# f-dangel/vivit

Measured on AMD Instinct MI355X. Metric: GGN eigenpairs/sec (Gram build + symeig), MLP 784-512-10, batch=4096, higher is better.
Workload: dtype f32

## Files before the change

### vivit_amd/csrc/sy2sb.hip

```cpp
#include <cstdlib>

#include "common.h"
#include "device_utils.h"
#include "eig_internal.h"

namespace vivit {

constexpr int SNB = 64;
constexpr int QT = 128;
constexpr int SGRP = 8;

__global__ __launch_bounds__(256) void sb_panel_load_kernel(const float *__restrict__ A, int64_t lda, int64_t j0, int64_t mp,
                                                            float *__restrict__ pan) {
  const int64_t idx = (int64_t)blockIdx.x * 256 + threadIdx.x;
  if (idx >= mp * SNB) return;
  const int64_t r = idx / SNB, c = idx - r * SNB;
  pan[idx] = A[(j0 + SNB + r) * lda + j0 + c];
}

__global__ __launch_bounds__(256) void sb_panel_load_row_kernel(const float *__restrict__ A, int64_t lda, int64_t j0, int64_t mp,
                                                                float *__restrict__ pan) {
  __shared__ float t[SNB][SNB + 1];
  const int64_t r0 = (int64_t)blockIdx.x * SNB;
  const int tid = threadIdx.x;
  for (int idx = tid; idx < SNB * SNB; idx += 256) {
    const int c = idx / SNB, rr = idx % SNB;
    t[c][rr] = r0 + rr < mp ? A[(j0 + c) * lda + j0 + SNB + r0 + rr] : 0.f;
  }
  __syncthreads();
  for (int idx = tid; idx < SNB * SNB; idx += 256) {
    const int rr = idx / SNB, c = idx % SNB;
    if (r0 + rr < mp) pan[(r0 + rr) * SNB + c] = t[c][rr];
  }
}

__global__ __launch_bounds__(256) void coef_gather_kernel(const float *__restrict__ S, int64_t lds_, int64_t g, int kp,
                                                          float *__restrict__ Coef) {
  const int idx = blockIdx.x * 256 + threadIdx.x;
  if (idx >= SNB * kp) return;
  const int k = idx / SNB, m = idx % SNB;
  Coef[(int64_t)m * kp + k] = S[(int64_t)k * lds_ + g + m];
}


__global__ __launch_bounds__(256) void qr_step_kernel(float *__restrict__ pan, int64_t mp, int c, int ncol, int nwg, QrPart pt,
                                                      float *__restrict__ vdst1, float *__restrict__ vdst2, int64_t lds_, int64_t gi0,
                                                      float *__restrict__ A, int64_t lda, int64_t j0,
                                                      float *__restrict__ tau1, float *__restrict__ betas) {
  __shared__ float tile[QT][SNB + 1];
  __shared__ float vs[QT], xs2[QT];
  __shared__ float zs[SNB];
  __shared__ float zq[4][SNB];
  __shared__ __attribute__((aligned(16))) float zq16[16][SNB];
  const int tid = threadIdx.x;
  const int64_t r0 = (int64_t)blockIdx.x * QT;
  constexpr int NTL = QT * (SNB / 4) / 256;
  float4 tl[NTL];
#pragma unroll
  for (int i = 0; i < NTL; ++i) {
    const int idx = tid + 256 * i;
    const int rl = idx / (SNB / 4), c4 = (idx - rl * (SNB / 4)) * 4;
    const int64_t r = r0 + rl;
    tl[i] = *reinterpret_cast<const float4 *>(pan + (r < mp ? r : 0) * SNB + c4);
  }
  const int par = c & 1;
  const float *uin = pt.u + (int64_t)par * nwg * SNB;
  const float *din = pt.diag + par * SNB;
  const int cq4 = tid & 15, q16 = tid >> 4;
  float4 pv[20];
#pragma unroll
  for (int i = 0; i < 20; ++i) {
    const int w = q16 + 16 * i;
    pv[i] = *reinterpret_cast<const float4 *>(uin + (int64_t)(w < nwg ? w : 0) * SNB + 4 * cq4);
  }
  const float din_c = din[c >= 0 ? c : 0], din_t = din[tid & (SNB - 1)];
  __builtin_amdgcn_sched_barrier(0);
#pragma unroll
  for (int i = 0; i < NTL; ++i) {
    const int idx = tid + 256 * i;
    const int rl = idx / (SNB / 4), c4 = (idx - rl * (SNB / 4)) * 4;
    const bool ok = r0 + rl < mp;
    tile[rl][c4 + 0] = ok ? tl[i].x : 0.f;
    tile[rl][c4 + 1] = ok ? tl[i].y : 0.f;
    tile[rl][c4 + 2] = ok ? tl[i].z : 0.f;
    tile[rl][c4 + 3] = ok ? tl[i].w : 0.f;
  }
  if (c >= 0) {
    {
      float4 acc = make_float4(0.f, 0.f, 0.f, 0.f);
#pragma unroll
      for (int i = 0; i < 20; ++i)
        if (q16 + 16 * i < nwg) { acc.x += pv[i].x; acc.y += pv[i].y; acc.z += pv[i].z; acc.w += pv[i].w; }
      for (int w0 = q16 + 16 * 20; w0 < nwg; w0 += 16 * 20) {
        float4 v[20];
#pragma unroll
        for (int i = 0; i < 20; ++i) {
          const int w = w0 + 16 * i;
          v[i] = *reinterpret_cast<const float4 *>(uin + (int64_t)(w < nwg ? w : 0) * SNB + 4 * cq4);
        }
#pragma unroll
        for (int i = 0; i < 20; ++i)
          if (w0 + 16 * i < nwg) { acc.x += v[i].x; acc.y += v[i].y; acc.z += v[i].z; acc.w += v[i].w; }
      }
      *reinterpret_cast<float4 *>(&zq16[q16][4 * cq4]) = acc;
    }
    __syncthreads();
    float ssq = 0.f;
#pragma unroll
    for (int g2 = 0; g2 < 16; ++g2) ssq += zq16[g2][c];
    const float alpha = din_c;
    float tau = 0.f, beta = alpha, scal = 0.f;
    if (ssq > 0.f) {
      beta = -copysignf(sqrt_nr(alpha * alpha + ssq), alpha);
      tau = (beta - alpha) * rcp_nr(beta);
      scal = rcp_nr(alpha - beta);
    }
    if (tid < SNB) {
      float u = 0.f;
#pragma unroll
      for (int g2 = 0; g2 < 16; ++g2) u += zq16[g2][tid];
      zs[tid] = tid > c ? tau * (din_t + scal * u) : 0.f;
    }
    if (tid < QT) {
      const int64_t r = r0 + tid;
      float v = 0.f;
      if (r < mp) {
        if (r == c) v = 1.f;
        else if (r > c) v = tile[tid][c] * scal;
        vdst1[(int64_t)c * lds_ + gi0 + r] = v;
        vdst2[(int64_t)c * lds_ + gi0 + r] = v;
        if (r >= c) A[(j0 + c) * lda + gi0 + r] = v;
      }
      vs[tid] = v;
    }
    if (blockIdx.x == 0 && tid == 0) { tau1[j0 + c] = tau; betas[c] = beta; }
  } else {
    if (tid < QT) vs[tid] = 0.f;
    if (tid < SNB) zs[tid] = 0.f;
  }
  __syncthreads();
  const int cn = c + 1;
  const bool has_next = cn < ncol;
  if (tid < QT) {
    const int64_t r = r0 + tid;
    xs2[tid] = (has_next && r > cn && r < mp) ? tile[tid][cn] - vs[tid] * zs[cn] : 0.f;
  }
  __syncthreads();
  {
    const int cc = tid & 63, q = tid >> 6;
    const float zc = zs[cc];
    float acc = 0.f;
#pragma unroll 8
    for (int i = 0; i < QT / 4; ++i) {
      const int rl = q + 4 * i;
      const float v = vs[rl];
      float x = tile[rl][cc];
      if (cc > c && v != 0.f) {
        x -= v * zc;
        tile[rl][cc] = x;
        if (r0 + rl < mp) pan[(r0 + rl) * SNB + cc] = x;
      }
      acc += xs2[rl] * x;
    }
    zq[q][cc] = acc;
  }
  if (!has_next) return;
  __syncthreads();
  {
    const int par = cn & 1;
    if (tid < SNB) pt.u[((int64_t)par * nwg + blockIdx.x) * SNB + tid] = (zq[0][tid] + zq[1][tid]) + (zq[2][tid] + zq[3][tid]);
    if (cn >= r0 && cn < r0 + QT && tid < SNB) pt.diag[par * SNB + tid] = tile[cn - r0][tid];
  }
}

constexpr int QP_WG = 32, QP_THREADS = 512;
struct QrPersistWs {
  float *ubuf;
  float *dbuf;
  int *counter;
  int *tmo;
  int attempt;
  int fault;
};

__device__ __forceinline__ float sel8(float a0, float a1, float a2, float a3, float a4, float a5, float a6, float a7, int j) {
  const float t0 = (j & 1) ? a1 : a0, t1 = (j & 1) ? a3 : a2, t2 = (j & 1) ? a5 : a4, t3 = (j & 1) ? a7 : a6;
  const float u0 = (j & 2) ? t1 : t0, u1 = (j & 2) ? t3 : t2;
  return (j & 4) ? u1 : u0;
}

template <int RI>
__global__ __launch_bounds__(QP_THREADS) void qr_persist_kernel(float *__restrict__ pan, int64_t mp, int ncol, QrPersistWs pw,
                                                                float *__restrict__ vdst1, float *__restrict__ vdst2, int64_t lds_,
                                                                int64_t gi0, float *__restrict__ A, int64_t lda, int64_t j0,
                                                                float *__restrict__ tau1, float *__restrict__ betas) {
  if ((blockIdx.x & 7) != 0) return;
  if (pw.attempt == 1 && __hip_atomic_load(pw.counter + 1, __ATOMIC_RELAXED, __HIP_MEMORY_SCOPE_AGENT) != PERSIST_ABORT) return;
  int *const cnt = pw.counter + 8 * pw.attempt;
  const int w = blockIdx.x >> 3;
  const int tid = threadIdx.x, lane = tid & 63, wave = tid >> 6;
  const int cg = tid & 7, rs = tid >> 3;
  constexpr int RW = 64 * RI;
  const int64_t rbase = (int64_t)w * RW;
  __shared__ float s_u[SNB], s_d[SNB], s_dn[SNB];
  __shared__ float s_red[QP_THREADS / 64][SNB];
  __shared__ float s_v[RW];
  __shared__ int s_flag[2];

  float x[RI][8];
#pragma unroll
  for (int i = 0; i < RI; ++i) {
    const int64_t r = rbase + rs + 64 * i;
    const float *src = pan + (r < mp ? r : 0) * SNB + 8 * cg;
    const float4 a = *reinterpret_cast<const float4 *>(src), b = *reinterpret_cast<const float4 *>(src + 4);
    const bool ok = r < mp;
    x[i][0] = ok ? a.x : 0.f; x[i][1] = ok ? a.y : 0.f; x[i][2] = ok ? a.z : 0.f; x[i][3] = ok ? a.w : 0.f;
    x[i][4] = ok ? b.x : 0.f; x[i][5] = ok ? b.y : 0.f; x[i][6] = ok ? b.z : 0.f; x[i][7] = ok ? b.w : 0.f;
  }
  if (tid == 0) {
    int xcc;
    __asm__ volatile("s_getreg_b32 %0, hwreg(HW_REG_XCC_ID)" : "=s"(xcc));
    __hip_atomic_store(pw.counter + 32 + w, xcc & 15, __ATOMIC_RELAXED, __HIP_MEMORY_SCOPE_AGENT);
    __asm__ volatile("s_waitcnt vmcnt(0)" ::: "memory");
    const bool go = persist_arrive(cnt, cnt + 1, QP_WG, ((pw.fault >> pw.attempt) & 1) ? 0ull : PERSIST_TIMEOUT_TICKS);
    const int dead = go ? 0 : 2;
    int slow = 0;
    const int x0 = __hip_atomic_load(pw.counter + 32, __ATOMIC_RELAXED, __HIP_MEMORY_SCOPE_AGENT);
    for (int i = 1; i < QP_WG; ++i) slow |= __hip_atomic_load(pw.counter + 32 + i, __ATOMIC_RELAXED, __HIP_MEMORY_SCOPE_AGENT) != x0;
    s_flag[0] = slow;
    s_flag[1] = dead;
  }
  __syncthreads();
  const bool slow = s_flag[0] != 0;
  if (s_flag[1] == 2) {
    if (tid == 0 && w == 0 && pw.attempt == 1) {
      __hip_atomic_fetch_or(pw.tmo, PERSIST_TMO_PANEL_QR, __ATOMIC_RELAXED, __HIP_MEMORY_SCOPE_AGENT);
      betas[0] = __builtin_nanf("");
    }
    return;
  }
  const int grp = lane & ~7;

  auto publish = [&](int cn) __attribute__((always_inline)) {
    float acc[8];
#pragma unroll
    for (int j = 0; j < 8; ++j) acc[j] = 0.f;
#pragma unroll
    for (int i = 0; i < RI; ++i) {
      const int64_t r = rbase + rs + 64 * i;
      float xn = __shfl(sel8(x[i][0], x[i][1], x[i][2], x[i][3], x[i][4], x[i][5], x[i][6], x[i][7], cn & 7), grp | (cn >> 3), 64);
      xn = (r > cn && r < mp) ? xn : 0.f;
#pragma unroll
      for (int j = 0; j < 8; ++j) acc[j] = fmaf(xn, x[i][j], acc[j]);
    }
#pragma unroll
    for (int j = 0; j < 8; ++j) {
      acc[j] += __shfl_xor(acc[j], 8, 64);
      acc[j] += __shfl_xor(acc[j], 16, 64);
      acc[j] += __shfl_xor(acc[j], 32, 64);
    }
    if (lane < 8) {
#pragma unroll
      for (int j = 0; j < 8; ++j) s_red[wave][8 * lane + j] = acc[j];
    }
    if (w == 0 && rs == cn) {
#pragma unroll
      for (int j = 0; j < 8; ++j) s_dn[8 * cg + j] = x[0][j];
    }
  };
  auto send = [&](int par) __attribute__((always_inline)) {
    if (wave == 0) {
      float u = 0.f;
#pragma unroll
      for (int q = 0; q < QP_THREADS / 64; ++q) u += s_red[q][lane];
      float *ub = pw.ubuf + ((size_t)par * QP_WG + w) * SNB + lane, *db = pw.dbuf + (size_t)par * SNB + lane;
      if (slow) {
        __hip_atomic_store(ub, u, __ATOMIC_RELAXED, __HIP_MEMORY_SCOPE_AGENT);
        if (w == 0) __hip_atomic_store(db, s_dn[lane], __ATOMIC_RELAXED, __HIP_MEMORY_SCOPE_AGENT);
      } else {
        *ub = u;
        if (w == 0) *db = s_dn[lane];
      }
      __asm__ volatile("s_waitcnt vmcnt(0)" ::: "memory");
      if (lane == 0) __hip_atomic_fetch_add(cnt, 1, __ATOMIC_RELAXED, __HIP_MEMORY_SCOPE_AGENT);
    }
  };

  publish(0);
  __syncthreads();
  send(0);
  for (int c = 0; c < ncol && !s_flag[1]; ++c) {
    const int par = c & 1;
    if (wave == 0) {
      const int target = (c + 2) * QP_WG;
      const unsigned long long t0 = __builtin_amdgcn_s_memrealtime();
      while (__hip_atomic_load(cnt, __ATOMIC_RELAXED, __HIP_MEMORY_SCOPE_AGENT) < target)
        if (__builtin_amdgcn_s_memrealtime() - t0 > PERSIST_TIMEOUT_TICKS) { s_flag[1] = 1; break; }
      const float *ub = pw.ubuf + (size_t)par * QP_WG * SNB + lane;
      float pv[QP_WG];
#pragma unroll
      for (int q = 0; q < QP_WG; ++q) pv[q] = __hip_atomic_load(ub + q * SNB, __ATOMIC_RELAXED, __HIP_MEMORY_SCOPE_AGENT);
      const float dn = __hip_atomic_load(pw.dbuf + (size_t)par * SNB + lane, __ATOMIC_RELAXED, __HIP_MEMORY_SCOPE_AGENT);
      float u = 0.f;
#pragma unroll
      for (int q = 0; q < QP_WG; ++q) u += pv[q];
      s_u[lane] = u;
      s_d[lane] = dn;
    }
    __syncthreads();
    if (s_flag[1]) break;
    const float ssq = s_u[c], alpha = s_d[c];
    float tau = 0.f, beta = alpha, scal = 0.f;
    if (ssq > 0.f) {
      beta = -copysignf(sqrt_nr(alpha * alpha + ssq), alpha);
      tau = (beta - alpha) * rcp_nr(beta);
      scal = rcp_nr(alpha - beta);
    }
    float z[8];
#pragma unroll
    for (int j = 0; j < 8; ++j) {
      const int cc = 8 * cg + j;
      z[j] = cc > c ? tau * (s_d[cc] + scal * s_u[cc]) : 0.f;
    }
#pragma unroll
    for (int i = 0; i < RI; ++i) {
      const int64_t r = rbase + rs + 64 * i;
      const float xc = __shfl(sel8(x[i][0], x[i][1], x[i][2], x[i][3], x[i][4], x[i][5], x[i][6], x[i][7], c & 7), grp | (c >> 3), 64);
      const float v = r == c ? 1.f : ((r > c && r < mp) ? xc * scal : 0.f);
      if (cg == 0) s_v[rs + 64 * i] = v;
#pragma unroll
      for (int j = 0; j < 8; ++j) x[i][j] = fmaf(-v, z[j], x[i][j]);
    }
    if (w == 0 && tid == 0) { tau1[j0 + c] = tau; betas[c] = beta; }
    const bool has_next = c + 1 < ncol;
    if (has_next) publish(c + 1);
    __syncthreads();
    if (has_next) send(par ^ 1);
    for (int idx = tid; idx < RW; idx += QP_THREADS) {
      const int64_t r = rbase + idx;
      if (r < mp) {
        const float v = s_v[idx];
        vdst1[(int64_t)c * lds_ + gi0 + r] = v;
        vdst2[(int64_t)c * lds_ + gi0 + r] = v;
        if (r >= c) A[(j0 + c) * lda + gi0 + r] = v;
      }
    }
  }
  if (w == 0) {
    const int64_t r = rs;
    if (r < mp) {
      float *dst = pan + r * SNB + 8 * cg;
      *reinterpret_cast<float4 *>(dst) = make_float4(x[0][0], x[0][1], x[0][2], x[0][3]);
      *reinterpret_cast<float4 *>(dst + 4) = make_float4(x[0][4], x[0][5], x[0][6], x[0][7]);
    }
    if (tid == 0 && s_flag[1]) {
      betas[0] = __builtin_nanf("");
      __hip_atomic_fetch_or(pw.tmo, PERSIST_TMO_PANEL_QR, __ATOMIC_RELAXED, __HIP_MEMORY_SCOPE_AGENT);
    }
  }
}

static bool qr_persist_enabled() {
  static int on = -1;
  if (on < 0) {
    const char *e = getenv("VIVIT_QR_PERSIST");
    on = e ? atoi(e) : 1;
  }
  return on != 0 && persist_override() != 0;
}
constexpr size_t QR_PERSIST_WS_BYTES = sizeof(float) * (2 * QP_WG * SNB + 2 * SNB) + 64 * sizeof(int) + 256;

static bool qr_persist_launch(float *pan, int64_t mp, int ncol, void *wsp, float *v1, float *v2, int64_t ldn, int64_t gi0, float *A,
                              int64_t lda, int64_t j0, float *tau1, float *betas, hipStream_t stream) {
  if (!qr_persist_enabled() || mp > (int64_t)QP_WG * 64 * 20 || device_cu_count() < 256) return false;
  QrPersistWs pw;
  pw.ubuf = reinterpret_cast<float *>(align_up(reinterpret_cast<uintptr_t>(wsp), 256));
  pw.dbuf = pw.ubuf + 2 * QP_WG * SNB;
  pw.counter = reinterpret_cast<int *>(pw.dbuf + 2 * SNB);
  pw.tmo = persist_timeout_word(stream);
  pw.fault = persist_fault();
  if (!pw.tmo) return false;
  if (hipMemsetAsync(pw.counter, 0, 64 * sizeof(int), stream) != hipSuccess) return false;
  const int64_t ri = cdiv(mp, (int64_t)QP_WG * 64);
  const dim3 grid(8 * QP_WG);
#define QP_LAUNCH(RI) qr_persist_kernel<RI><<<grid, QP_THREADS, 0, stream>>>(pan, mp, ncol, pw, v1, v2, ldn, gi0, A, lda, j0, tau1, betas)
  for (int attempt = 0; attempt < 2; ++attempt) {
    pw.attempt = attempt;
    if (ri <= 1) QP_LAUNCH(1);
    else if (ri <= 2) QP_LAUNCH(2);
    else if (ri <= 3) QP_LAUNCH(3);
    else if (ri <= 5) QP_LAUNCH(5);
    else if (ri <= 8) QP_LAUNCH(8);
    else if (ri <= 12) QP_LAUNCH(12);
    else if (ri <= 16) QP_LAUNCH(16);
    else QP_LAUNCH(20);
  }
#undef QP_LAUNCH
  return true;
}

struct Sk64Args {
  const float *Coef;
  const float *B;
  float *Out;
  int64_t ldcoef, ldb, ldo, N;
  int K;
  float alpha, beta;
};
constexpr int SK_LDC = 36, SK_COLS = 128, SK_LDB = SK_COLS + 4, SK_NT = SK_COLS / 64;

__global__ __launch_bounds__(256) void skinny64_kernel(Sk64Args p) {
  __shared__ __attribute__((aligned(16))) float sC[64 * SK_LDC];
  __shared__ __attribute__((aligned(16))) float sB[32 * SK_LDB];
  const int tid = threadIdx.x, lane = tid & 63, wave = tid >> 6;
  const int r = lane & 31, h = lane >> 5, wm = wave >> 1, wn = wave & 1;
  const int64_t c0 = (int64_t)blockIdx.x * SK_COLS;
  f32x16 acc[SK_NT];
#pragma unroll
  for (int t = 0; t < SK_NT; ++t)
#pragma unroll
    for (int e = 0; e < 16; ++e) acc[t][e] = 0.f;
  constexpr int NLB = 32 * SK_COLS / 4 / 256;
  float4 rc[2], rb[NLB];
  auto gload = [&](int k0) __attribute__((always_inline)) {
#pragma unroll
    for (int i = 0; i < 2; ++i) {
      const int idx = tid + 256 * i;
      const int m = idx >> 3, kq = (idx & 7) * 4;
      rc[i] = *reinterpret_cast<const float4 *>(p.Coef + (int64_t)m * p.ldcoef + k0 + kq);
    }
#pragma unroll
    for (int i = 0; i < NLB; ++i) {
      const int idx = tid + 256 * i;
      const int kr = idx / (SK_COLS / 4), cq = (idx % (SK_COLS / 4)) * 4;
      const int64_t c = c0 + cq;
      rb[i] = *reinterpret_cast<const float4 *>(p.B + (int64_t)(k0 + kr) * p.ldb + (c < p.N ? c : 0));
    }
    __builtin_amdgcn_sched_barrier(0);
  };
  gload(0);
  for (int k0 = 0; k0 < p.K; k0 += 32) {
    __syncthreads();
#pragma unroll
    for (int i = 0; i < 2; ++i) {
      const int idx = tid + 256 * i;
      *reinterpret_cast<float4 *>(sC + (idx >> 3) * SK_LDC + (idx & 7) * 4) = rc[i];
    }
#pragma unroll
    for (int i = 0; i < NLB; ++i) {
      const int idx = tid + 256 * i;
      const int kr = idx / (SK_COLS / 4), cq = (idx % (SK_COLS / 4)) * 4;
      *reinterpret_cast<float4 *>(sB + kr * SK_LDB + cq) = c0 + cq < p.N ? rb[i] : make_float4(0.f, 0.f, 0.f, 0.f);
    }
    __syncthreads();
    if (k0 + 32 < p.K) gload(k0 + 32);
    const float *pa = sC + (32 * wm + r) * SK_LDC + 4 * h;
#pragma unroll
    for (int j = 0; j < 4; ++j) {
      const float4 a4 = *reinterpret_cast<const float4 *>(pa + 8 * j);
      const float av[4] = {a4.x, a4.y, a4.z, a4.w};
      float bv[4][SK_NT];
#pragma unroll
      for (int i = 0; i < 4; ++i)
#pragma unroll
        for (int t = 0; t < SK_NT; ++t) bv[i][t] = sB[(8 * j + 4 * h + i) * SK_LDB + 64 * wn + 32 * t + r];
#pragma unroll
      for (int i = 0; i < 4; ++i)
#pragma unroll
        for (int t = 0; t < SK_NT; ++t) acc[t] = __builtin_amdgcn_mfma_f32_32x32x2f32(av[i], bv[i][t], acc[t], 0, 0, 0);
    }
  }
#pragma unroll
  for (int t = 0; t < SK_NT; ++t) {
    const int64_t c = c0 + 64 * wn + 32 * t + r;
    if (c < p.N) {
#pragma unroll
      for (int e = 0; e < 16; ++e) {
        const int m = 32 * wm + (e & 3) + 8 * (e >> 2) + 4 * h;
        float *o = p.Out + (int64_t)m * p.ldo + c;
        float v = p.alpha * acc[t][e];
        if (p.beta != 0.f) v += p.beta * *o;
        *o = v;
      }
    }
  }
}

static bool skinny64_launch(const float *Coef, int64_t ldcoef, const float *B, int64_t ldb, float *Out, int64_t ldo, int64_t N, int64_t K,
                            float alpha, float beta, hipStream_t stream) {
  if (K < 32 || K % 32 != 0 || K > 4096 || N % 4 != 0 || ldb % 4 != 0 || ldcoef % 4 != 0 ||
      (reinterpret_cast<uintptr_t>(Coef) & 15) || (reinterpret_cast<uintptr_t>(B) & 15))
    return false;
  Sk64Args a;
  a.Coef = Coef; a.B = B; a.Out = Out; a.ldcoef = ldcoef; a.ldb = ldb; a.ldo = ldo; a.N = N; a.K = (int)K; a.alpha = alpha; a.beta = beta;
  skinny64_kernel<<<(unsigned)cdiv(N, SK_COLS), 256, 0, stream>>>(a);
  return true;
}

__global__ __launch_bounds__(256) void w_coef_kernel(const float *__restrict__ T, const float *__restrict__ G, float *__restrict__ Coef) {
  __shared__ float sT[SNB][SNB + 1], sG[SNB][SNB + 1], sU[SNB][SNB + 1];
  const int tid = threadIdx.x, lane = tid & 63, wave = tid >> 6;
  const int r = lane & 31, h = lane >> 5, qi = (wave >> 1) * 32, qj = (wave & 1) * 32;
  for (int idx = tid; idx < SNB * SNB; idx += 256) {
    sT[idx / SNB][idx % SNB] = T[idx];
    sG[idx / SNB][idx % SNB] = G[idx];
  }
  __syncthreads();
  f32x16 acc;
#pragma unroll
  for (int e = 0; e < 16; ++e) acc[e] = 0.f;
#pragma unroll 8
  for (int s2 = 0; s2 < SNB / 2; ++s2) acc = __builtin_amdgcn_mfma_f32_32x32x2f32(sT[2 * s2 + h][qi + r], sG[2 * s2 + h][qj + r], acc, 0, 0, 0);
#pragma unroll
  for (int e = 0; e < 16; ++e) sU[qi + (e & 3) + 8 * (e >> 2) + 4 * h][qj + r] = acc[e];
  __syncthreads();
#pragma unroll
  for (int e = 0; e < 16; ++e) acc[e] = 0.f;
#pragma unroll 8
  for (int s2 = 0; s2 < SNB / 2; ++s2) acc = __builtin_amdgcn_mfma_f32_32x32x2f32(sU[qi + r][2 * s2 + h], sT[2 * s2 + h][qj + r], acc, 0, 0, 0);
#pragma unroll
  for (int e = 0; e < 16; ++e) {
    const int a_ = qi + (e & 3) + 8 * (e >> 2) + 4 * h, b_ = qj + r;
    Coef[a_ * 2 * SNB + b_] = -0.5f * acc[e];
    Coef[a_ * 2 * SNB + SNB + b_] = sT[b_][a_];
  }
}

__global__ __launch_bounds__(256) void sb_panel_store_kernel(float *__restrict__ A, int64_t lda, int64_t j0, int64_t mp,
                                                             const float *__restrict__ pan, const float *__restrict__ betas) {
  const int idx = blockIdx.x * 256 + threadIdx.x;
  if (idx >= SNB * SNB) return;
  const int r = idx / SNB, c = idx - r * SNB;
  if (r >= mp) return;
  A[(j0 + SNB + r) * lda + j0 + c] = (r < c) ? pan[(int64_t)r * SNB + c] : (r == c ? betas[c] : 0.f);
}

__global__ __launch_bounds__(256) void larft_kernel(const float *__restrict__ S, int64_t lds_, const float *__restrict__ tau, int nb,
                                                    int nvalid, float *__restrict__ T) {
  constexpr int H = SNB / 2, LD = SNB + 1;
  __shared__ float Ss[SNB * LD], Ts[SNB * LD], Xs[H * (H + 1)], taus[SNB];
  const int tid = threadIdx.x;
  for (int idx = tid; idx < SNB * SNB; idx += 256) {
    Ss[(idx / SNB) * LD + (idx % SNB)] = S[(int64_t)(idx / SNB) * lds_ + (idx % SNB)];
    Ts[(idx / SNB) * LD + (idx % SNB)] = 0.f;
  }
  if (tid < SNB) taus[tid] = (tid < nvalid && tid < nb) ? tau[tid] : 0.f;
  __syncthreads();
  if (tid < SNB) {
    const int half = tid / H, j = tid % H;
    const float *Sb = Ss + half * (H * LD + H), *tb = taus + half * H;
    float t[H];
#pragma unroll
    for (int c = 0; c < H; ++c) t[c] = 0.f;
#pragma unroll
    for (int i = H - 1; i >= 0; --i) {
      float acc = 0.f;
#pragma unroll
      for (int c = i + 1; c < H; ++c) acc += Sb[i * LD + c] * t[c];
      t[i] = i == j ? tb[j] : (i < j ? -tb[i] * acc : 0.f);
    }
    float *Tb = Ts + half * (H * LD + H);
#pragma unroll
    for (int i = 0; i < H; ++i) Tb[i * LD + j] = t[i];
  }
  __syncthreads();
  if (tid < 64) {
    const int r = tid & 31, h = tid >> 5;
    f32x16 acc;
#pragma unroll
    for (int e = 0; e < 16; ++e) acc[e] = 0.f;
#pragma unroll 8
    for (int s2 = 0; s2 < H / 2; ++s2)
      acc = __builtin_amdgcn_mfma_f32_32x32x2f32(Ss[r * LD + H + 2 * s2 + h], Ts[(H + 2 * s2 + h) * LD + H + r], acc, 0, 0, 0);
#pragma unroll
    for (int e = 0; e < 16; ++e) Xs[((e & 3) + 8 * (e >> 2) + 4 * h) * (H + 1) + r] = acc[e];
  }
  __syncthreads();
  if (tid < 64) {
    const int r = tid & 31, h = tid >> 5;
    f32x16 acc;
#pragma unroll
    for (int e = 0; e < 16; ++e) acc[e] = 0.f;
#pragma unroll 8
    for (int s2 = 0; s2 < H / 2; ++s2)
      acc = __builtin_amdgcn_mfma_f32_32x32x2f32(Ts[r * LD + 2 * s2 + h], Xs[(2 * s2 + h) * (H + 1) + r], acc, 0, 0, 0);
#pragma unroll
    for (int e = 0; e < 16; ++e) Ts[((e & 3) + 8 * (e >> 2) + 4 * h) * LD + H + r] = -acc[e];
  }
  __syncthreads();
  for (int idx = tid; idx < SNB * SNB; idx += 256) T[idx] = Ts[(idx / SNB) * LD + (idx % SNB)];
}

__global__ __launch_bounds__(256) void sb_extract_band_kernel(const float *__restrict__ A, int64_t lda, int64_t n,
                                                              float *__restrict__ AB, int64_t ldab) {
  const int64_t idx = (int64_t)blockIdx.x * 256 + threadIdx.x;
  if (idx >= n * ldab) return;
  const int64_t i = idx / ldab;
  const int d = (int)(idx - i * ldab);
  const int64_t j = i - 2 * SNB + d;
  AB[idx] = (d >= SNB && d <= 2 * SNB && j >= 0) ? A[i * lda + j] : 0.f;
}

static size_t sy2sb_gemm_ws_bytes(int64_t n) {
  size_t m = 0;
  for (int64_t mp = 1; mp <= n; mp = mp < 4096 ? mp * 2 : mp + 4096) {
    const int64_t q = mp < n ? mp : n;
    size_t a = gemm_workspace_bytes(SNB, SNB, q, false);
    size_t b = gemm_workspace_bytes(SNB, q, q, false);
    size_t c = gemm_workspace_bytes(SNB, q, SNB, false);
    size_t d = 0, e = 0, f = 0;
    for (int g = 1; g < SGRP; ++g) {
      const size_t d1 = gemm_workspace_bytes(SNB, 2 * SNB * g + SNB, q, false), e1 = gemm_workspace_bytes(SNB, q, 2 * SNB * g, false);
      const size_t f1 = gemm_workspace_bytes(q, SNB, 2 * SNB * g, false);
      d = d1 > d ? d1 : d; e = e1 > e ? e1 : e; f = f1 > f ? f1 : f;
    }
    m = a > m ? a : m; m = b > m ? b : m; m = c > m ? c : m;
    m = d > m ? d : m; m = e > m ? e : m; m = f > m ? f : m;
    const size_t u = gemm_workspace_bytes(q, q, (int64_t)2 * SNB * SGRP, true);
    m = u > m ? u : m;
  }
  size_t a = gemm_workspace_bytes(SNB, SNB, n, false), b = gemm_workspace_bytes(SNB, n, n, false);
  m = a > m ? a : m; m = b > m ? b : m;
  return m * 2;
}

Sy2sbWs sy2sb_layout(Arena &a, int64_t n) {
  const int64_t nwg = cdiv(n, QT) + 1;
  Sy2sbWs ws;
  ws.pan = a.take<float>(n * SNB);
  ws.stackA = a.take<float>(2 * SGRP * SNB * n);
  ws.stackB = a.take<float>(2 * SGRP * SNB * n);
  ws.xt = a.take<float>(SNB * n);
  ws.G12 = a.take<float>(SNB * 2 * SNB * SGRP);
  ws.qp.u = a.take<float>(2 * nwg * SNB);
  ws.qp.diag = a.take<float>(2 * SNB);
  ws.qpw = a.take<char>(QR_PERSIST_WS_BYTES);
  ws.S = a.take<float>(SNB * SNB);
  ws.T = a.take<float>(SNB * SNB);
  ws.Y3 = a.take<float>(SNB * SNB);
  ws.S2 = a.take<float>(SNB * SNB);
  ws.tau1 = a.take<float>(n);
  ws.betas = a.take<float>(SNB);
  ws.gws_bytes = sy2sb_gemm_ws_bytes(n);
  ws.gws = a.take<char>(ws.gws_bytes);
  return ws;
}

size_t sy2sb_workspace_bytes(int64_t n) {
  Arena m;
  sy2sb_layout(m, n);
  return m.used() + 1024;
}

int sy2sb_launch(float *A, int64_t n, int64_t lda, const Sy2sbWs &ws, hipStream_t stream) {
  if (hipMemsetAsync(ws.tau1, 0, sizeof(float) * n, stream) != hipSuccess) return VIVIT_E_LAUNCH;

  const int64_t ldn = n;
  const bool rowmode = (n % 4 == 0) && (lda % 4 == 0) && (reinterpret_cast<uintptr_t>(A) & 15) == 0;
  auto factor_panel = [&](int64_t j0, float *v1, float *v2) -> int {
    const int64_t mp = n - j0 - SNB, gi0 = j0 + SNB;
    const int ncol = (int)(mp < SNB ? mp : SNB);
    const int g = (int)cdiv(mp, QT);
    if (rowmode) sb_panel_load_row_kernel<<<(unsigned)cdiv(mp, SNB), 256, 0, stream>>>(A, lda, j0, mp, ws.pan);
    else sb_panel_load_kernel<<<(unsigned)cdiv(mp * SNB, 256), 256, 0, stream>>>(A, lda, j0, mp, ws.pan);
    if (!qr_persist_launch(ws.pan, mp, ncol, ws.qpw, v1, v2, ldn, gi0, A, lda, j0, ws.tau1, ws.betas, stream))
      for (int c = -1; c < ncol; ++c)
        qr_step_kernel<<<g, 256, 0, stream>>>(ws.pan, mp, c, ncol, g, ws.qp, v1, v2, ldn, gi0, A, lda, j0, ws.tau1, ws.betas);
    sb_panel_store_kernel<<<(unsigned)cdiv(SNB * SNB, 256), 256, 0, stream>>>(A, lda, j0, mp, ws.pan, ws.betas);
    return launch_status();
  };
  auto compute_w = [&](int64_t j0, float *Vt, float *Wt, float *Wcopy, int64_t kp, const float *sAg, const float *sBg) -> int {
    const int64_t mp = n - j0 - SNB, gi0 = j0 + SNB;
    const int ncol = (int)(mp < SNB ? mp : SNB);
    float *A22 = A + gi0 * lda + gi0;
    int st;
    prof_mark(PROF_STAGE_SY2SB, stream);
    st = gemm_launch(LAY_K, LAY_M, Vt, A22, Wt, SNB, mp, mp, ldn, lda, ldn, 1.f, 0.f, false, ws.gws, ws.gws_bytes, stream);
    prof_mark(PROF_STAGE_SY2SB_PP, stream);
    if (st != VIVIT_OK) return st;
    const int64_t ldg = kp + SNB;
    st = gemm_launch(LAY_K, LAY_K, Vt, sAg, ws.G12, SNB, ldg, mp, ldn, ldn, ldg, 1.f, 0.f, false, ws.gws, ws.gws_bytes, stream);
    if (st != VIVIT_OK) return st;
    larft_kernel<<<1, 256, 0, stream>>>(ws.G12 + kp, ldg, ws.tau1 + j0, SNB, ncol, ws.T);
    if (kp > 0) {
      if (!skinny64_launch(ws.G12, ldg, sBg, ldn, Wt, ldn, mp, kp, -1.f, 1.f, stream)) {
        st = gemm_launch(LAY_K, LAY_M, ws.G12, sBg, Wt, SNB, mp, kp, ldg, ldn, ldn, -1.f, 1.f, false, ws.gws, ws.gws_bytes, stream);
        if (st != VIVIT_OK) return st;
      }
    }
    st = gemm_launch(LAY_K, LAY_K, Wt, Vt, ws.S2, SNB, SNB, mp, ldn, ldn, SNB, 1.f, 0.f, false, ws.gws, ws.gws_bytes, stream);
    if (st != VIVIT_OK) return st;
    w_coef_kernel<<<1, 256, 0, stream>>>(ws.T, ws.S2, ws.G12);
    if (Wt == Vt + (int64_t)SNB * ldn &&
        skinny64_launch(ws.G12, 2 * SNB, Vt, ldn, Wcopy, ldn, mp, 2 * SNB, 1.f, 0.f, stream))
      return hipMemcpy2DAsync(Wt, sizeof(float) * ldn, Wcopy, sizeof(float) * ldn, sizeof(float) * mp, SNB, hipMemcpyDeviceToDevice,
                              stream) == hipSuccess ? VIVIT_OK : VIVIT_E_LAUNCH;
    float *Xt = ws.xt + gi0;
    st = gemm_launch(LAY_M, LAY_M, ws.T, Wt, Xt, SNB, mp, SNB, SNB, ldn, ldn, 1.f, 0.f, false, ws.gws, ws.gws_bytes, stream);
    if (st != VIVIT_OK) return st;
    if (hipMemcpy2DAsync(Wt, sizeof(float) * ldn, Xt, sizeof(float) * ldn, sizeof(float) * mp, SNB, hipMemcpyDeviceToDevice,
                         stream) != hipSuccess)
      return VIVIT_E_LAUNCH;
    st = gemm_launch(LAY_K, LAY_M, ws.G12, Vt, Wt, SNB, mp, SNB, 2 * SNB, ldn, ldn, 1.f, 1.f, false, ws.gws, ws.gws_bytes, stream);
    if (st != VIVIT_OK) return st;
    return hipMemcpy2DAsync(Wcopy, sizeof(float) * ldn, Wt, sizeof(float) * ldn, sizeof(float) * mp, SNB, hipMemcpyDeviceToDevice,
                            stream) == hipSuccess ? VIVIT_OK : VIVIT_E_LAUNCH;
  };

  float *sA = ws.stackA, *sB = ws.stackB;
  for (int64_t j0 = 0; j0 + SNB < n;) {
    int st;
    if (hipMemsetAsync(sA, 0, sizeof(float) * 2 * SGRP * SNB * n, stream) != hipSuccess) return VIVIT_E_LAUNCH;
    if (hipMemsetAsync(sB, 0, sizeof(float) * 2 * SGRP * SNB * n, stream) != hipSuccess) return VIVIT_E_LAUNCH;
    int np = 0;
    int64_t gi_last = 0;
    for (; np < SGRP && j0 + SNB < n; ++np, j0 += SNB) {
      const int64_t gi = j0 + SNB;
      const int64_t kp = (int64_t)2 * SNB * np;
      if (np > 0) {
        const int64_t gc = gi - SNB;
        bool done = false;
        if (rowmode) {
          coef_gather_kernel<<<(unsigned)cdiv(SNB * kp, 256), 256, 0, stream>>>(sA, ldn, gc, (int)kp, ws.G12);
          done = skinny64_launch(ws.G12, kp, sB + gc, ldn, A + gc * lda + gc, lda, n - gc, kp, -1.f, 1.f, stream);
        }
        if (!done) {
          if (rowmode) return VIVIT_E_UNSUPPORTED;
          st = gemm_launch(LAY_M, LAY_M, sA + gc, sB + gc, A + gc * lda + gc, n - gc, SNB, kp, ldn, ldn, lda, -1.f, 1.f, false,
                           ws.gws, ws.gws_bytes, stream);
          if (st != VIVIT_OK) return st;
        }
      }
      float *Vrow = sA + kp * n, *Wrow = sA + (kp + SNB) * n;
      st = factor_panel(j0, Vrow, sB + (kp + SNB) * n);
      if (st != VIVIT_OK) return st;
      st = compute_w(j0, Vrow + gi, Wrow + gi, sB + kp * n + gi, kp, sA + gi, sB + gi);
      if (st != VIVIT_OK) return st;
      gi_last = gi;
    }
    const int64_t mt = n - gi_last;
    prof_mark(PROF_STAGE_SY2SB, stream);
    st = gemm_launch(LAY_M, LAY_M, sA + gi_last, sB + gi_last, A + gi_last * lda + gi_last, mt, mt, (int64_t)2 * SNB * np, ldn, ldn,
                     lda, -1.f, 1.f, true, ws.gws, ws.gws_bytes, stream);
    prof_mark(PROF_STAGE_SY2SB_UPD, stream);
    if (st != VIVIT_OK) return st;
  }
  return launch_status();
}

struct PanelQrWs {
  QrPart qp;
  float *S;
  void *qpw, *gws;
  size_t gws_bytes;
};

static PanelQrWs panel_qr_layout(Arena &a, int64_t mp) {
  const int64_t nwg = cdiv(mp, QT) + 1;
  PanelQrWs ws;
  ws.qp.u = a.take<float>(2 * nwg * SNB);
  ws.qp.diag = a.take<float>(2 * SNB);
  ws.S = a.take<float>(SNB * SNB);
  ws.qpw = a.take<char>(QR_PERSIST_WS_BYTES);
  ws.gws_bytes = gemm_workspace_bytes(SNB, SNB, mp, false);
  ws.gws = a.take<char>(ws.gws_bytes);
  return ws;
}

size_t sy2sb_panel_qr_workspace_bytes(int64_t mp) {
  Arena m;
  panel_qr_layout(m, mp);
  return m.used() + 1024;
}

int sy2sb_panel_qr_launch(float *pan, int64_t mp, float *Vt, int64_t ldv, float *tau, float *betas, float *T, void *wsbase,
                          size_t ws_bytes, hipStream_t stream) {
  if (ws_bytes < sy2sb_panel_qr_workspace_bytes(mp)) return VIVIT_E_WORKSPACE;
  Arena a(wsbase, ws_bytes);
  const PanelQrWs ws = panel_qr_layout(a, mp);
  if (a.overflow()) return VIVIT_E_WORKSPACE;
  const QrPart qp = ws.qp;
  float *S = ws.S;
  void *qpw = ws.qpw, *gws = ws.gws;
  const size_t gws_bytes = ws.gws_bytes;
  const int ncol = (int)(mp < SNB ? mp : SNB);
  const int g = (int)cdiv(mp, QT);
  if (hipMemsetAsync(tau, 0, sizeof(float) * SNB, stream) != hipSuccess) return VIVIT_E_LAUNCH;
  if (hipMemsetAsync(betas, 0, sizeof(float) * SNB, stream) != hipSuccess) return VIVIT_E_LAUNCH;
  if (hipMemset2DAsync(Vt, sizeof(float) * ldv, 0, sizeof(float) * mp, SNB, stream) != hipSuccess) return VIVIT_E_LAUNCH;
  if (!qr_persist_launch(pan, mp, ncol, qpw, Vt, Vt, ldv, 0, Vt, ldv, 0, tau, betas, stream))
    for (int c = -1; c < ncol; ++c)
      qr_step_kernel<<<g, 256, 0, stream>>>(pan, mp, c, ncol, g, qp, Vt, Vt, ldv, 0, Vt, ldv, 0, tau, betas);
  int st = gemm_launch(LAY_K, LAY_K, Vt, Vt, S, SNB, SNB, mp, ldv, ldv, SNB, 1.f, 0.f, false, gws, gws_bytes, stream);
  if (st != VIVIT_OK) return st;
  larft_kernel<<<1, 256, 0, stream>>>(S, SNB, tau, SNB, ncol, T);
  return launch_status();
}

int sy2sb_extract_band_launch(const float *A, int64_t lda, int64_t n, float *AB, int64_t ldab, hipStream_t stream) {
  sb_extract_band_kernel<<<(unsigned)cdiv(n * ldab, 256), 256, 0, stream>>>(A, lda, n, AB, ldab);
  return launch_status();
}

}

using namespace vivit;

extern "C" {

size_t vivit_sy2sb_f32_workspace_bytes(int64_t n) { return n > 0 ? sy2sb_workspace_bytes(n) : 0; }

int vivit_sy2sb_f32(float *A, int64_t n, int64_t lda, float *AB, float *tau1, void *workspace, size_t workspace_bytes,
                    void *stream) {
  if (n < 1 || !A || !AB || !tau1 || lda < n) return VIVIT_E_BADARG;
  if (!workspace || workspace_bytes < sy2sb_workspace_bytes(n)) return VIVIT_E_WORKSPACE;
  hipStream_t s = static_cast<hipStream_t>(stream);
  Arena a(workspace, workspace_bytes);
  const Sy2sbWs ws = sy2sb_layout(a, n);
  if (a.overflow()) return VIVIT_E_WORKSPACE;
  int st = sy2sb_launch(A, n, lda, ws, s);
  if (st != VIVIT_OK) return st;
  st = sy2sb_extract_band_launch(A, lda, n, AB, 2 * SNB + 1, s);
  if (st != VIVIT_OK) return st;
  if (hipMemcpyAsync(tau1, ws.tau1, sizeof(float) * n, hipMemcpyDeviceToDevice, s) != hipSuccess) return VIVIT_E_LAUNCH;
  return VIVIT_OK;
}

size_t vivit_sy2sb_panel_qr_f32_workspace_bytes(int64_t mp) { return mp > 0 ? sy2sb_panel_qr_workspace_bytes(mp) : 0; }

int vivit_sy2sb_panel_qr_f32(float *pan, int64_t mp, float *Vt, int64_t ldv, float *tau, float *betas, float *T, void *workspace,
                             size_t workspace_bytes, void *stream) {
  if (mp < 1 || !pan || !Vt || !tau || !betas || !T || ldv < mp) return VIVIT_E_BADARG;
  if (!workspace) return VIVIT_E_WORKSPACE;
  return sy2sb_panel_qr_launch(pan, mp, Vt, ldv, tau, betas, T, workspace, workspace_bytes, static_cast<hipStream_t>(stream));
}

}
```

Before: 7467.

## Fuse panel-store, counter reset and W copy into persistent QR kernels

The persistent panel-QR kernel now writes the R factor (betas on the diagonal and the upper triangle) straight into A, so the separate panel-store kernel is skipped on that path. The counter memset is folded into the panel-load kernel, and the skinny GEMM writes a second output so the trailing 2D device-to-device memcpy is gone. The QR inner loop is also reworked to use packed f32x2 FMAs and a single ds_bpermute broadcast per column that is reused for the reflector update, and it moves V stores off wave 0. The aim is fewer launches and copies per panel and less per-column ALU work, at the cost of more complex kernel code and extra NaN-propagation handling.

```diff
diff --git a/vivit_amd/csrc/sy2sb.hip b/vivit_amd/csrc/sy2sb.hip
--- a/vivit_amd/csrc/sy2sb.hip
+++ b/vivit_amd/csrc/sy2sb.hip
@@ -11,7 +11,8 @@
 constexpr int SGRP = 8;
 
 __global__ __launch_bounds__(256) void sb_panel_load_kernel(const float *__restrict__ A, int64_t lda, int64_t j0, int64_t mp,
-                                                            float *__restrict__ pan) {
+                                                            float *__restrict__ pan, int *__restrict__ qcnt) {
+  if (blockIdx.x == 0 && threadIdx.x < 64) qcnt[threadIdx.x] = 0;
   const int64_t idx = (int64_t)blockIdx.x * 256 + threadIdx.x;
   if (idx >= mp * SNB) return;
   const int64_t r = idx / SNB, c = idx - r * SNB;
@@ -19,10 +20,11 @@
 }
 
 __global__ __launch_bounds__(256) void sb_panel_load_row_kernel(const float *__restrict__ A, int64_t lda, int64_t j0, int64_t mp,
-                                                                float *__restrict__ pan) {
+                                                                float *__restrict__ pan, int *__restrict__ qcnt) {
   __shared__ float t[SNB][SNB + 1];
   const int64_t r0 = (int64_t)blockIdx.x * SNB;
   const int tid = threadIdx.x;
+  if (blockIdx.x == 0 && tid < 64) qcnt[tid] = 0;
   for (int idx = tid; idx < SNB * SNB; idx += 256) {
     const int c = idx / SNB, rr = idx % SNB;
     t[c][rr] = r0 + rr < mp ? A[(j0 + c) * lda + j0 + SNB + r0 + rr] : 0.f;
@@ -183,17 +185,15 @@
   int fault;
 };
 
-__device__ __forceinline__ float sel8(float a0, float a1, float a2, float a3, float a4, float a5, float a6, float a7, int j) {
-  const float t0 = (j & 1) ? a1 : a0, t1 = (j & 1) ? a3 : a2, t2 = (j & 1) ? a5 : a4, t3 = (j & 1) ? a7 : a6;
-  const float u0 = (j & 2) ? t1 : t0, u1 = (j & 2) ? t3 : t2;
-  return (j & 4) ? u1 : u0;
-}
+typedef float f32x2 __attribute__((ext_vector_type(2)));
+__device__ __forceinline__ float *qp_at(float *base, unsigned i) { return reinterpret_cast<float *>(reinterpret_cast<char *>(base) + (i << 2)); }
 
 template <int RI>
 __global__ __launch_bounds__(QP_THREADS) void qr_persist_kernel(float *__restrict__ pan, int64_t mp, int ncol, QrPersistWs pw,
                                                                 float *__restrict__ vdst1, float *__restrict__ vdst2, int64_t lds_,
                                                                 int64_t gi0, float *__restrict__ A, int64_t lda, int64_t j0,
-                                                                float *__restrict__ tau1, float *__restrict__ betas) {
+                                                                float *__restrict__ tau1, float *__restrict__ betas,
+                                                                float *__restrict__ Rdst, int64_t ldr) {
   if ((blockIdx.x & 7) != 0) return;
   if (pw.attempt == 1 && __hip_atomic_load(pw.counter + 1, __ATOMIC_RELAXED, __HIP_MEMORY_SCOPE_AGENT) != PERSIST_ABORT) return;
   int *const cnt = pw.counter + 8 * pw.attempt;
@@ -202,20 +202,22 @@
   const int cg = tid & 7, rs = tid >> 3;
   constexpr int RW = 64 * RI;
   const int64_t rbase = (int64_t)w * RW;
-  __shared__ float s_u[SNB], s_d[SNB], s_dn[SNB];
-  __shared__ float s_red[QP_THREADS / 64][SNB];
-  __shared__ float s_v[RW];
+  const int r0 = w * RW + rs, mpi = (int)mp;
+  __shared__ float s_all[3 * SNB + QP_THREADS + RW];
+  float *const s_u = s_all, *const s_d = s_all + SNB, *const s_dn = s_all + 2 * SNB, *const s_v = s_all + 3 * SNB + QP_THREADS;
+  float (*const s_red)[SNB] = reinterpret_cast<float (*)[SNB]>(s_all + 3 * SNB);
   __shared__ int s_flag[2];
 
-  float x[RI][8];
+  f32x2 x[RI][4];
+  float xb[RI];
 #pragma unroll
   for (int i = 0; i < RI; ++i) {
     const int64_t r = rbase + rs + 64 * i;
     const float *src = pan + (r < mp ? r : 0) * SNB + 8 * cg;
     const float4 a = *reinterpret_cast<const float4 *>(src), b = *reinterpret_cast<const float4 *>(src + 4);
     const bool ok = r < mp;
-    x[i][0] = ok ? a.x : 0.f; x[i][1] = ok ? a.y : 0.f; x[i][2] = ok ? a.z : 0.f; x[i][3] = ok ? a.w : 0.f;
-    x[i][4] = ok ? b.x : 0.f; x[i][5] = ok ? b.y : 0.f; x[i][6] = ok ? b.z : 0.f; x[i][7] = ok ? b.w : 0.f;
+    x[i][0][0] = ok ? a.x : 0.f; x[i][0][1] = ok ? a.y : 0.f; x[i][1][0] = ok ? a.z : 0.f; x[i][1][1] = ok ? a.w : 0.f;
+    x[i][2][0] = ok ? b.x : 0.f; x[i][2][1] = ok ? b.y : 0.f; x[i][3][0] = ok ? b.z : 0.f; x[i][3][1] = ok ? b.w : 0.f;
   }
   if (tid == 0) {
     int xcc;
@@ -236,36 +238,51 @@
     if (tid == 0 && w == 0 && pw.attempt == 1) {
       __hip_atomic_fetch_or(pw.tmo, PERSIST_TMO_PANEL_QR, __ATOMIC_RELAXED, __HIP_MEMORY_SCOPE_AGENT);
       betas[0] = __builtin_nanf("");
+      if (Rdst) Rdst[0] = __builtin_nanf("");
     }
     return;
   }
   const int grp = lane & ~7;
 
   auto publish = [&](int cn) __attribute__((always_inline)) {
-    float acc[8];
-#pragma unroll
-    for (int j = 0; j < 8; ++j) acc[j] = 0.f;
+    const int src = (grp | (cn >> 3)) << 2;
+    switch (cn & 7) {
+#define QP_BCAST(K)                                                                                                  \
+  case K:                                                                                                            \
+    _Pragma("unroll") for (int i = 0; i < RI; ++i)                                                                   \
+      xb[i] = __int_as_float(__builtin_amdgcn_ds_bpermute(src, __float_as_int(x[i][K >> 1][K & 1])));               \
+    break;
+      QP_BCAST(0) QP_BCAST(1) QP_BCAST(2) QP_BCAST(3) QP_BCAST(4) QP_BCAST(5) QP_BCAST(6) QP_BCAST(7)
+#undef QP_BCAST
+    }
+    f32x2 acc[4];
+#pragma unroll
+    for (int jj = 0; jj < 4; ++jj) acc[jj] = f32x2{0.f, 0.f};
 #pragma unroll
     for (int i = 0; i < RI; ++i) {
-      const int64_t r = rbase + rs + 64 * i;
-      float xn = __shfl(sel8(x[i][0], x[i][1], x[i][2], x[i][3], x[i][4], x[i][5], x[i][6], x[i][7], cn & 7), grp | (cn >> 3), 64);
-      xn = (r > cn && r < mp) ? xn : 0.f;
-#pragma unroll
-      for (int j = 0; j < 8; ++j) acc[j] = fmaf(xn, x[i][j], acc[j]);
-    }
-#pragma unroll
-    for (int j = 0; j < 8; ++j) {
-      acc[j] += __shfl_xor(acc[j], 8, 64);
-      acc[j] += __shfl_xor(acc[j], 16, 64);
-      acc[j] += __shfl_xor(acc[j], 32, 64);
-    }
+      const int r = r0 + 64 * i;
+      const float xn = (r > cn && r < mpi) ? xb[i] : 0.f;
+      const f32x2 xn2 = {xn, xn};
+#pragma unroll
+      for (int jj = 0; jj < 4; ++jj) acc[jj] = __builtin_elementwise_fma(xn2, x[i][jj], acc[jj]);
+    }
+#pragma unroll
+    for (int jj = 0; jj < 4; ++jj)
+#pragma unroll
+      for (int e = 0; e < 2; ++e) {
+        float a = acc[jj][e];
+        a += __shfl_xor(a, 8, 64);
+        a += __shfl_xor(a, 16, 64);
+        a += __shfl_xor(a, 32, 64);
+        acc[jj][e] = a;
+      }
     if (lane < 8) {
 #pragma unroll
-      for (int j = 0; j < 8; ++j) s_red[wave][8 * lane + j] = acc[j];
+      for (int jj = 0; jj < 4; ++jj) { s_red[wave][8 * lane + 2 * jj] = acc[jj][0]; s_red[wave][8 * lane + 2 * jj + 1] = acc[jj][1]; }
     }
     if (w == 0 && rs == cn) {
 #pragma unroll
-      for (int j = 0; j < 8; ++j) s_dn[8 * cg + j] = x[0][j];
+      for (int jj = 0; jj < 4; ++jj) { s_dn[8 * cg + 2 * jj] = x[0][jj][0]; s_dn[8 * cg + 2 * jj + 1] = x[0][jj][1]; }
     }
   };
   auto send = [&](int par) __attribute__((always_inline)) {
@@ -273,13 +290,13 @@
       float u = 0.f;
 #pragma unroll
       for (int q = 0; q < QP_THREADS / 64; ++q) u += s_red[q][lane];
-      float *ub = pw.ubuf + ((size_t)par * QP_WG + w) * SNB + lane, *db = pw.dbuf + (size_t)par * SNB + lane;
+      float *const ub = pw.ubuf + (par * QP_WG + w) * SNB, *const db = pw.dbuf + par * SNB;
       if (slow) {
-        __hip_atomic_store(ub, u, __ATOMIC_RELAXED, __HIP_MEMORY_SCOPE_AGENT);
-        if (w == 0) __hip_atomic_store(db, s_dn[lane], __ATOMIC_RELAXED, __HIP_MEMORY_SCOPE_AGENT);
+        __hip_atomic_store(qp_at(ub, lane), u, __ATOMIC_RELAXED, __HIP_MEMORY_SCOPE_AGENT);
+        if (w == 0) __hip_atomic_store(qp_at(db, lane), s_dn[lane], __ATOMIC_RELAXED, __HIP_MEMORY_SCOPE_AGENT);
       } else {
-        *ub = u;
-        if (w == 0) *db = s_dn[lane];
+        *qp_at(ub, lane) = u;
+        if (w == 0) *qp_at(db, lane) = s_dn[lane];
       }
       __asm__ volatile("s_waitcnt vmcnt(0)" ::: "memory");
       if (lane == 0) __hip_atomic_fetch_add(cnt, 1, __ATOMIC_RELAXED, __HIP_MEMORY_SCOPE_AGENT);
@@ -296,11 +313,11 @@
       const unsigned long long t0 = __builtin_amdgcn_s_memrealtime();
       while (__hip_atomic_load(cnt, __ATOMIC_RELAXED, __HIP_MEMORY_SCOPE_AGENT) < target)
         if (__builtin_amdgcn_s_memrealtime() - t0 > PERSIST_TIMEOUT_TICKS) { s_flag[1] = 1; break; }
-      const float *ub = pw.ubuf + (size_t)par * QP_WG * SNB + lane;
+      float *const ub = pw.ubuf + par * QP_WG * SNB;
       float pv[QP_WG];
 #pragma unroll
-      for (int q = 0; q < QP_WG; ++q) pv[q] = __hip_atomic_load(ub + q * SNB, __ATOMIC_RELAXED, __HIP_MEMORY_SCOPE_AGENT);
-      const float dn = __hip_atomic_load(pw.dbuf + (size_t)par * SNB + lane, __ATOMIC_RELAXED, __HIP_MEMORY_SCOPE_AGENT);
+      for (int q = 0; q < QP_WG; ++q) pv[q] = __hip_atomic_load(qp_at(ub, q * SNB + lane), __ATOMIC_RELAXED, __HIP_MEMORY_SCOPE_AGENT);
+      const float dn = __hip_atomic_load(qp_at(pw.dbuf + par * SNB, lane), __ATOMIC_RELAXED, __HIP_MEMORY_SCOPE_AGENT);
       float u = 0.f;
 #pragma unroll
       for (int q = 0; q < QP_WG; ++q) u += pv[q];
@@ -316,33 +333,42 @@
       tau = (beta - alpha) * rcp_nr(beta);
       scal = rcp_nr(alpha - beta);
     }
-    float z[8];
+    f32x2 z[4];
 #pragma unroll
     for (int j = 0; j < 8; ++j) {
       const int cc = 8 * cg + j;
-      z[j] = cc > c ? tau * (s_d[cc] + scal * s_u[cc]) : 0.f;
+      z[j >> 1][j & 1] = cc > c ? tau * (s_d[cc] + scal * s_u[cc]) : 0.f;
     }
 #pragma unroll
     for (int i = 0; i < RI; ++i) {
-      const int64_t r = rbase + rs + 64 * i;
-      const float xc = __shfl(sel8(x[i][0], x[i][1], x[i][2], x[i][3], x[i][4], x[i][5], x[i][6], x[i][7], c & 7), grp | (c >> 3), 64);
-      const float v = r == c ? 1.f : ((r > c && r < mp) ? xc * scal : 0.f);
+      const int r = r0 + 64 * i;
+      const float v = r == c ? 1.f : ((r > c && r < mpi) ? xb[i] * scal : 0.f);
       if (cg == 0) s_v[rs + 64 * i] = v;
-#pragma unroll
-      for (int j = 0; j < 8; ++j) x[i][j] = fmaf(-v, z[j], x[i][j]);
-    }
-    if (w == 0 && tid == 0) { tau1[j0 + c] = tau; betas[c] = beta; }
+      const f32x2 nv = {-v, -v};
+#pragma unroll
+      for (int jj = 0; jj < 4; ++jj) x[i][jj] = __builtin_elementwise_fma(nv, z[jj], x[i][jj]);
+    }
+    if (w == 0 && tid == 64) {
+      tau1[j0 + c] = tau;
+      betas[c] = beta;
+      if (Rdst) Rdst[c * ldr + c] = beta;
+    }
     const bool has_next = c + 1 < ncol;
     if (has_next) publish(c + 1);
     __syncthreads();
     if (has_next) send(par ^ 1);
-    for (int idx = tid; idx < RW; idx += QP_THREADS) {
-      const int64_t r = rbase + idx;
-      if (r < mp) {
-        const float v = s_v[idx];
-        vdst1[(int64_t)c * lds_ + gi0 + r] = v;
-        vdst2[(int64_t)c * lds_ + gi0 + r] = v;
-        if (r >= c) A[(j0 + c) * lda + gi0 + r] = v;
+    if (wave != 0) {
+      const int64_t ob = (int64_t)c * lds_ + gi0 + rbase;
+      float *const d1 = vdst1 + ob, *const d2 = vdst2 + ob, *const da = A + (j0 + c) * lda + gi0 + rbase;
+      const int rb = w * RW;
+      for (unsigned idx = tid - 64; idx < (unsigned)RW; idx += QP_THREADS - 64) {
+        const int r = rb + (int)idx;
+        if (r < mpi) {
+          const float v = s_v[idx];
+          *qp_at(d1, idx) = v;
+          *qp_at(d2, idx) = v;
+          if (r >= c) *qp_at(da, idx) = v;
+        }
       }
     }
   }
@@ -350,11 +376,19 @@
     const int64_t r = rs;
     if (r < mp) {
       float *dst = pan + r * SNB + 8 * cg;
-      *reinterpret_cast<float4 *>(dst) = make_float4(x[0][0], x[0][1], x[0][2], x[0][3]);
-      *reinterpret_cast<float4 *>(dst + 4) = make_float4(x[0][4], x[0][5], x[0][6], x[0][7]);
+      *reinterpret_cast<float4 *>(dst) = make_float4(x[0][0][0], x[0][0][1], x[0][1][0], x[0][1][1]);
+      *reinterpret_cast<float4 *>(dst + 4) = make_float4(x[0][2][0], x[0][2][1], x[0][3][0], x[0][3][1]);
+    }
+    if (Rdst && r < mp) {
+#pragma unroll
+      for (int j = 0; j < 8; ++j) {
+        const int cc = 8 * cg + j;
+        if (cc != rs) Rdst[r * ldr + cc] = rs < cc ? x[0][j >> 1][j & 1] : 0.f;
+      }
     }
     if (tid == 0 && s_flag[1]) {
       betas[0] = __builtin_nanf("");
+      if (Rdst) Rdst[0] = __builtin_nanf("");
       __hip_atomic_fetch_or(pw.tmo, PERSIST_TMO_PANEL_QR, __ATOMIC_RELAXED, __HIP_MEMORY_SCOPE_AGENT);
     }
   }
@@ -370,20 +404,26 @@
 }
 constexpr size_t QR_PERSIST_WS_BYTES = sizeof(float) * (2 * QP_WG * SNB + 2 * SNB) + 64 * sizeof(int) + 256;
 
-static bool qr_persist_launch(float *pan, int64_t mp, int ncol, void *wsp, float *v1, float *v2, int64_t ldn, int64_t gi0, float *A,
-                              int64_t lda, int64_t j0, float *tau1, float *betas, hipStream_t stream) {
-  if (!qr_persist_enabled() || mp > (int64_t)QP_WG * 64 * 20 || device_cu_count() < 256) return false;
-  QrPersistWs pw;
+static QrPersistWs qr_persist_ws(void *wsp) {
+  QrPersistWs pw = {};
   pw.ubuf = reinterpret_cast<float *>(align_up(reinterpret_cast<uintptr_t>(wsp), 256));
   pw.dbuf = pw.ubuf + 2 * QP_WG * SNB;
   pw.counter = reinterpret_cast<int *>(pw.dbuf + 2 * SNB);
+  return pw;
+}
+
+static bool qr_persist_launch(float *pan, int64_t mp, int ncol, void *wsp, bool zeroed, float *v1, float *v2, int64_t ldn, int64_t gi0,
+                              float *A, int64_t lda, int64_t j0, float *tau1, float *betas, float *Rdst, int64_t ldr,
+                              hipStream_t stream) {
+  if (!qr_persist_enabled() || mp > (int64_t)QP_WG * 64 * 20 || device_cu_count() < 256) return false;
+  QrPersistWs pw = qr_persist_ws(wsp);
   pw.tmo = persist_timeout_word(stream);
   pw.fault = persist_fault();
   if (!pw.tmo) return false;
-  if (hipMemsetAsync(pw.counter, 0, 64 * sizeof(int), stream) != hipSuccess) return false;
+  if (!zeroed && hipMemsetAsync(pw.counter, 0, 64 * sizeof(int), stream) != hipSuccess) return false;
   const int64_t ri = cdiv(mp, (int64_t)QP_WG * 64);
   const dim3 grid(8 * QP_WG);
-#define QP_LAUNCH(RI) qr_persist_kernel<RI><<<grid, QP_THREADS, 0, stream>>>(pan, mp, ncol, pw, v1, v2, ldn, gi0, A, lda, j0, tau1, betas)
+#define QP_LAUNCH(RI) qr_persist_kernel<RI><<<grid, QP_THREADS, 0, stream>>>(pan, mp, ncol, pw, v1, v2, ldn, gi0, A, lda, j0, tau1, betas, Rdst, ldr)
   for (int attempt = 0; attempt < 2; ++attempt) {
     pw.attempt = attempt;
     if (ri <= 1) QP_LAUNCH(1);
@@ -403,7 +443,8 @@
   const float *Coef;
   const float *B;
   float *Out;
-  int64_t ldcoef, ldb, ldo, N;
+  float *Out2;
+  int64_t ldcoef, ldb, ldo, ldo2, N;
   int K;
   float alpha, beta;
 };
@@ -481,18 +522,19 @@
         float v = p.alpha * acc[t][e];
         if (p.beta != 0.f) v += p.beta * *o;
         *o = v;
+        if (p.Out2) p.Out2[(int64_t)m * p.ldo2 + c] = v;
       }
     }
   }
 }
 
 static bool skinny64_launch(const float *Coef, int64_t ldcoef, const float *B, int64_t ldb, float *Out, int64_t ldo, int64_t N, int64_t K,
-                            float alpha, float beta, hipStream_t stream) {
+                            float alpha, float beta, hipStream_t stream, float *Out2 = nullptr, int64_t ldo2 = 0) {
   if (K < 32 || K % 32 != 0 || K > 4096 || N % 4 != 0 || ldb % 4 != 0 || ldcoef % 4 != 0 ||
       (reinterpret_cast<uintptr_t>(Coef) & 15) || (reinterpret_cast<uintptr_t>(B) & 15))
     return false;
   Sk64Args a;
-  a.Coef = Coef; a.B = B; a.Out = Out; a.ldcoef = ldcoef; a.ldb = ldb; a.ldo = ldo; a.N = N; a.K = (int)K; a.alpha = alpha; a.beta = beta;
+  a.Coef = Coef; a.B = B; a.Out = Out; a.Out2 = Out2; a.ldo2 = ldo2; a.ldcoef = ldcoef; a.ldb = ldb; a.ldo = ldo; a.N = N; a.K = (int)K; a.alpha = alpha; a.beta = beta;
   skinny64_kernel<<<(unsigned)cdiv(N, SK_COLS), 256, 0, stream>>>(a);
   return true;
 }
@@ -661,12 +703,15 @@
     const int64_t mp = n - j0 - SNB, gi0 = j0 + SNB;
     const int ncol = (int)(mp < SNB ? mp : SNB);
     const int g = (int)cdiv(mp, QT);
-    if (rowmode) sb_panel_load_row_kernel<<<(unsigned)cdiv(mp, SNB), 256, 0, stream>>>(A, lda, j0, mp, ws.pan);
-    else sb_panel_load_kernel<<<(unsigned)cdiv(mp * SNB, 256), 256, 0, stream>>>(A, lda, j0, mp, ws.pan);
-    if (!qr_persist_launch(ws.pan, mp, ncol, ws.qpw, v1, v2, ldn, gi0, A, lda, j0, ws.tau1, ws.betas, stream))
+    int *const qcnt = qr_persist_ws(ws.qpw).counter;
+    if (rowmode) sb_panel_load_row_kernel<<<(unsigned)cdiv(mp, SNB), 256, 0, stream>>>(A, lda, j0, mp, ws.pan, qcnt);
+    else sb_panel_load_kernel<<<(unsigned)cdiv(mp * SNB, 256), 256, 0, stream>>>(A, lda, j0, mp, ws.pan, qcnt);
+    if (!qr_persist_launch(ws.pan, mp, ncol, ws.qpw, true, v1, v2, ldn, gi0, A, lda, j0, ws.tau1, ws.betas, A + gi0 * lda + j0, lda,
+                           stream)) {
       for (int c = -1; c < ncol; ++c)
         qr_step_kernel<<<g, 256, 0, stream>>>(ws.pan, mp, c, ncol, g, ws.qp, v1, v2, ldn, gi0, A, lda, j0, ws.tau1, ws.betas);
-    sb_panel_store_kernel<<<(unsigned)cdiv(SNB * SNB, 256), 256, 0, stream>>>(A, lda, j0, mp, ws.pan, ws.betas);
+      sb_panel_store_kernel<<<(unsigned)cdiv(SNB * SNB, 256), 256, 0, stream>>>(A, lda, j0, mp, ws.pan, ws.betas);
+    }
     return launch_status();
   };
   auto compute_w = [&](int64_t j0, float *Vt, float *Wt, float *Wcopy, int64_t kp, const float *sAg, const float *sBg) -> int {
@@ -692,9 +737,8 @@
     if (st != VIVIT_OK) return st;
     w_coef_kernel<<<1, 256, 0, stream>>>(ws.T, ws.S2, ws.G12);
     if (Wt == Vt + (int64_t)SNB * ldn &&
-        skinny64_launch(ws.G12, 2 * SNB, Vt, ldn, Wcopy, ldn, mp, 2 * SNB, 1.f, 0.f, stream))
-      return hipMemcpy2DAsync(Wt, sizeof(float) * ldn, Wcopy, sizeof(float) * ldn, sizeof(float) * mp, SNB, hipMemcpyDeviceToDevice,
-                              stream) == hipSuccess ? VIVIT_OK : VIVIT_E_LAUNCH;
+        skinny64_launch(ws.G12, 2 * SNB, Vt, ldn, Wcopy, ldn, mp, 2 * SNB, 1.f, 0.f, stream, Wt, ldn))
+      return VIVIT_OK;
     float *Xt = ws.xt + gi0;
     st = gemm_launch(LAY_M, LAY_M, ws.T, Wt, Xt, SNB, mp, SNB, SNB, ldn, ldn, 1.f, 0.f, false, ws.gws, ws.gws_bytes, stream);
     if (st != VIVIT_OK) return st;
@@ -788,7 +832,7 @@
   if (hipMemsetAsync(tau, 0, sizeof(float) * SNB, stream) != hipSuccess) return VIVIT_E_LAUNCH;
   if (hipMemsetAsync(betas, 0, sizeof(float) * SNB, stream) != hipSuccess) return VIVIT_E_LAUNCH;
   if (hipMemset2DAsync(Vt, sizeof(float) * ldv, 0, sizeof(float) * mp, SNB, stream) != hipSuccess) return VIVIT_E_LAUNCH;
-  if (!qr_persist_launch(pan, mp, ncol, qpw, Vt, Vt, ldv, 0, Vt, ldv, 0, tau, betas, stream))
+  if (!qr_persist_launch(pan, mp, ncol, qpw, false, Vt, Vt, ldv, 0, Vt, ldv, 0, tau, betas, nullptr, 0, stream))
     for (int c = -1; c < ncol; ++c)
       qr_step_kernel<<<g, 256, 0, stream>>>(pan, mp, c, ncol, g, qp, Vt, Vt, ldv, 0, Vt, ldv, 0, tau, betas);
   int st = gemm_launch(LAY_K, LAY_K, Vt, Vt, S, SNB, SNB, mp, ldv, ldv, SNB, 1.f, 0.f, false, gws, gws_bytes, stream);
```

After: 7523, median of 6. Within noise of the previous version (+0.8%).
